# kalekundert/addapt

Measured on AMD Instinct MI355X. Metric: MC steps/sec (fold+score+accept), 100-nt sgRNA, 4096 walkers, 1/8 GPU, higher is better.
Workload: dtype i16x2; 1 GPU; BASELINE configs[1] (MFE-fold score only): default objective (apo: not active, holo: active; THEO aptamer 0.32 uM), 4 minimum-free-energy folds per scored step, synthetic 100-nt sgRNA template (SURVEY.md 8d), 4096 walkers per GPU, annealing 5 to 0 in 300 steps; fold=mfe, bppm=False, walkers_per_gpu=4096, global_walkers=4096, length=100, parallelism=walker-sharded x1 (no data-path collective)

## Files before the change

addapt_amd/csrc/mfe_pair.hip:

```cpp
#include <hip/hip_runtime.h>

#include <algorithm>
#include <cstdint>
#include <cstdio>
#include <cstdlib>
#include <utility>

#include "dev_types.hpp"
#include "fold_common.hpp"
#include "launch.hpp"
#include "mfe_common.hpp"

namespace adx {

#define PSTAMP(k) ADX_STAMP_AT(k)
#ifdef ADX_STAMP
#define PSTAMP_PARAMS , unsigned long long *st_acc, unsigned long long &st_last
#define PSTAMP_ARGS , st_acc, st_last
__device__ unsigned long long g_stamps_p[16][16];
__device__ unsigned long long g_stamps_pe[16][16];
#else
#define PSTAMP_PARAMS
#define PSTAMP_ARGS
#endif
// ... 145 lines not shown
        if (!ok[q]) continue;
        L.cc[off(d, N) + i - 1] = static_cast<uint8_t>(rtype(ty[q]) * 25 + (wjp[q] & 7) * 5 + (wim[q] & 7));
        u32 h = INF16;
        if (((wi1[q] >> 8) & 255) >= uint32_t(u)) {
            h = padd(hv[q], f1[q]);
            if (u == 3 || u == 4 || u == 6) {
                const int sh = special_hp(spk, hp_key(L.S, i, u + 2));
                if (sh >= 0) h = spv[sh];
            }
        }
        if (d == mL - 1 && mL > 0 && mt[q]) h = pmin(h, mextra);
        if (inb[q]) {
            L.qbm[off(d, N) + i - 1] = pr[q] ? h : MARK16;
            L.qm1[colb(j) + i - 1] = pr[q] ? f2[q] : INF16;
        }
    }
}

template <int NT, int NM>
__device__ __forceinline__ void pair_constants(const DevScaled *__restrict__ XS, const DevTables *__restrict__ TT,
                                               const CP &L) {
    static_assert(NT >= 288 && NT >= MFE_E4_SLOTS * 4, "one table element per thread");
    const int tid = threadIdx.x;
    const u32 *gct = reinterpret_cast<const u32 *>(XS->ctab);
    constexpr int NCT = (CT_SIZE + NT - 1) / NT;
    u32 v_ct[NCT];
#pragma unroll
    for (int t = 0; t < NCT; t++) v_ct[t] = gct[min(tid + t * NT, CT_SIZE - 1)];
    const DevTables &T0 = *TT;
    const u32 v_mh = __float_as_uint((&T0.mmH[0][0][0])[min(tid, 199)]);
    const u32 v_mi = __float_as_uint((&T0.mmI[0][0][0])[min(tid, 199)]);
    const u32 v_ms = __float_as_uint((&T0.mlstem[0][0][0])[min(tid, 199)]);
    const u32 v_ex = __float_as_uint((&T0.ext[0][0][0])[min(tid, 287)]);
    const u32 v_tau = __float_as_uint(T0.termAU[tid & 7]);
    const int ke = min(tid, MFE_E4_SLOTS * 4 - 1);
    const int e4a = MFE_E4_A[ke >> 2][ke & 3], e4u = MFE_E4_U[ke >> 2];
    const u32 v_e4 = XS->ku16[e4u][max(e4a, 0)];
#pragma unroll
    for (int t = 0; t < NCT; t++)
        if (tid + t * NT < CT_SIZE) L.ct[tid + t * NT] = v_ct[t];
    if (tid < 200) {
        L.dt[DT_MMH + tid] = v_mh;
        L.dt[DT_MMI + tid] = v_mi;
        L.dt[DT_MLS + tid] = v_ms;
    }
    if (tid < 288) L.dt[DT_EXT + tid] = v_ex;
    if (tid < 8) L.dt[DT_TAU + tid] = v_tau;
    if (tid < MFE_E4_SLOTS * 4) L.e4[tid] = e4a < 0 ? INF16 : v_e4;
    for (int k = tid; k < NM - 3; k += NT) {
        (L.qbm - (NM - 3))[k] = INF16;
        (L.cc - (NM - 3))[k] = 0;
    }
}

template <int NT, int NM>
__device__ __forceinline__ bool pair_setup(const KArgs &ka, const DevScaled *__restrict__ XS,
                                           const DevTables *__restrict__ TT, const int *vs, const uint8_t *raw,
                                           const CP &L, const IncM &inc, const int tid,
                                           unsigned long long *sst) {
    static_assert(NT == NWV * WAVE, "one wave per block slot");
    DevVariant V = ka.variants[vs[0]];
    V.ctx = uni(V.ctx), V.cons_off = uni(V.cons_off);
    const bool mh0 = uni(V.motif) != 0, mh1 = uni(ka.variants[vs[1]].motif) != 0;
    const int N = uni(V.N);
    const int lane = tid & (WAVE - 1);
    const int wid = uni(tid / WAVE);
    const int NP = L.np;
#ifdef ADX_STAMP
    const unsigned long long st_setup0 = __builtin_amdgcn_s_memtime();
#endif
    const Band bd = inc.band(N);
    const bool incr = bd.incr;
    const int m_lo = bd.m_lo;

    static_assert(NT >= MAX_SPECIAL_HP && NT >= MAX_MOTIF && NT >= NM + 2, "one setup element per thread");
    const u32 v_hp = __float_as_uint(XS->hp[min(tid, N)]);
    const int n_sp = uni(XS->n_special);
    const uint32_t v_spk = XS->sp_key[min(tid, MAX_SPECIAL_HP - 1)];
    const u32 v_spv = __float_as_uint(XS->sp_val[min(tid, MAX_SPECIAL_HP - 1)]);
    const uint8_t v_mc = XS->motif_code[min(tid, MAX_MOTIF - 1)];
    const int8_t v_mp = XS->motif_pt[min(tid, MAX_MOTIF - 1)];
    const uint8_t *cons = ka.cons + V.cons_off;
    const int np = N + 2;
    const int kp = min(tid, np - 1);
    uint8_t v_sw, v_up, v_dn, v_pt, v_en, v_fl;
    {
        const uint8_t *bef = nullptr, *aft = nullptr;
        int blen = 0;
        if (V.ctx >= 0) {
            bef = ka.ctx_seq + ka.ctx_off[4 * V.ctx + 0];
            blen = ka.ctx_off[4 * V.ctx + 1];
            aft = ka.ctx_seq + ka.ctx_off[4 * V.ctx + 2];
        }
        const int pp = (kp == 0 ? N : (kp == N + 1 ? 1 : kp)) - 1;
        const uint8_t *sp = pp < blen ? bef + pp : (pp < blen + ka.Nraw ? raw + (pp - blen) : aft + (pp - blen - ka.Nraw));
        v_sw = *sp;
        v_up = cons[kp];
        v_dn = cons[np + kp];
        v_pt = cons[2 * np + kp];
        v_en = cons[3 * np + kp];
        v_fl = cons[4 * np + kp];
    }
    if (tid < np) {
        L.S[tid] = v_sw;
        L.up[tid] = v_up;
        L.dn[tid] = v_dn;
        L.ptn[tid] = v_pt;
        L.enc[tid] = v_en;
        L.flg[tid] = v_fl;
        L.mat[tid] = 0;
        L.pos[tid] = u32(v_sw) | (u32(v_fl & 7) << 3) | (u32(v_up) << 8) | (u32(v_pt) << 16) | (u32(v_en) << 24);
    }
    const bool cst = tid >= 1 && tid <= N && (v_fl || v_pt);
    u32 *hpf = L.colmin;
    static_assert(4 * (NM + 2) >= NM + 1, "hairpin factors fit the U slots");
    if (tid <= N) hpf[tid] = v_hp;
    uint32_t *spk = reinterpret_cast<uint32_t *>(L.part);
    u32 *spv = spk + MAX_SPECIAL_HP;
    uint8_t *mcode = reinterpret_cast<uint8_t *>(spk + 2 * MAX_SPECIAL_HP);
    int8_t *mpt = reinterpret_cast<int8_t *>(mcode + MAX_MOTIF);
    static_assert(2 * MAX_SPECIAL_HP * 4 + 2 * MAX_MOTIF <= PLay<NM>::MLA - PLay<NM>::PART, "setup tables fit the partials");
    if (tid < MAX_SPECIAL_HP) {
        const bool on = tid < n_sp;
        spk[tid] = on ? v_spk : 0xFFFFFFFFu;
        spv[tid] = on ? v_spv : INF16;
    }
    if (tid < MAX_MOTIF) {
        mcode[tid] = v_mc;
        mpt[tid] = v_mp;
    }

    constexpr int CNM = ((NM - 4) * (NM - 3)) >> 1;
    constexpr int RS = (3 * (CNM >> 1) + NT - 1) / NT;
    const int Crs = ((N - 4) * (N - 3)) >> 1, half = Crs >> 1;
    uint2 rsv[RS];
    constexpr int RC = (((CNM + 15) >> 4) + NT - 1) / NT;
    const int C16 = (Crs + 15) >> 4;
    uint4 rcv[RC];
    u32 rod = 0, r5 = 0;
    if (incr) {
        const size_t Cs = size_t(ka.cells);
        const size_t gap = Cs - size_t(2 * half);
#pragma unroll
        for (int t = 0; t < RS; t++) {
            const int k = tid + t * NT;
            const int kk = k < 3 * half ? k : 0;
            const size_t o = size_t(2 * kk) + (kk >= half ? gap : 0) + (kk >= 2 * half ? gap : 0);
            rsv[t] = *reinterpret_cast<const uint2 *>(inc.src + o);
        }
#pragma unroll
        for (int t = 0; t < RC; t++) {
            const int k = tid + t * NT;
            rcv[t] = inc.cc_src[k < C16 ? k : 0];
        }
        rod = inc.src[min(tid, 2) * Cs + max(Crs - 1, 0)];
        r5 = inc.src[3 * Cs + min(tid, N)];
    } else {
        const int C = ((N - 4) * (N - 3)) >> 1;
        for (int k = tid; k < C; k += NT) L.qm[k] = INF16;
    }
#ifdef ADX_STAMP
    const unsigned long long st_s1 = __builtin_amdgcn_s_memtime();
#endif
    const bool constrained = block_or(L.flag, cst);
    const int mL = uni(XS->motif_len);
#ifdef ADX_STAMP
    const unsigned long long st_s2 = __builtin_amdgcn_s_memtime();
#endif
    if ((mh0 || mh1) && mL > 0) {
        for (int o0 = 1 + wid * WAVE; o0 + mL - 1 <= N; o0 += NT) {
            const int o = o0 + lane;
            const bool in = o + mL - 1 <= N;
            bool ok = in;
            for (int k0 = 0; k0 < mL; k0 += 8) {
                uint32_t sb[8], mb[8];
#pragma unroll
                for (int t = 0; t < 8; t++) {
                    sb[t] = L.S[min(o + k0 + t, N + 1)];
                    mb[t] = mcode[k0 + t];
                }
#pragma unroll
                for (int t = 0; t < 8; t++) ok = ok && (k0 + t >= mL || sb[t] == mb[t]);
                if (__ballot(ok) == 0) break;
            }
            if (in) L.mat[o] = ok ? 1 : 0;
        }
        __syncthreads();
        motif_constraints(L, mpt, mL, N, wid, lane);
    }
#ifdef ADX_STAMP
    const unsigned long long st_s25 = __builtin_amdgcn_s_memtime();
#endif
    if (incr) {
        static_assert(PLay<NM>::QM - PLay<NM>::QBM == PLay<NM>::QM1 - PLay<NM>::QM, "one stride between the tables");
        const int gapl = int((PLay<NM>::QM - PLay<NM>::QBM) / 4) - 2 * half;
#pragma unroll
        for (int t = 0; t < RS; t++) {
            const int k = tid + t * NT;
            if (k < 3 * half) {
                const int o = 2 * k + (k >= half ? gapl : 0) + (k >= 2 * half ? gapl : 0);
                *reinterpret_cast<uint2 *>(L.qbm + o) = rsv[t];
            }
        }
        if ((Crs & 1) && tid < 3) (tid == 0 ? L.qbm : tid == 1 ? L.qm : L.qm1)[Crs - 1] = rod;
#pragma unroll
        for (int t = 0; t < RC; t++) {
            const int k = tid + t * NT;
            if (k < C16) reinterpret_cast<uint4 *>(L.cc)[k] = rcv[t];
        }
        if (tid <= m_lo - 2 && tid <= N) L.q5[tid] = r5;
    }
    static_assert(NM - 4 <= 2 * WAVE, "the diagonals' quarter-set counts in two lane-sets");
    static_assert((NM - 4) + ((NM - 4) * (NM - 3) / 2 + 15) / 16 <= 6 * (NM + 2), "quarter-sets fit the split slots");
    u32 *qtab = L.mla;
    int tot = 0;
#pragma unroll
    for (int xs = 0; xs < 2; xs++) {
        const int d = 4 + xs * WAVE + lane;
        const int n = d <= N - 1 ? max(0, bd.chi(d) - bd.clo(d) + 1) : 0;
        const int q = (n + 15) >> 4;
        int v = q;
#pragma unroll
        for (int o = 1; o < WAVE; o <<= 1) {
            const int t = __shfl_up(v, o, WAVE);
            if (lane >= o) v += t;
        }
        if (wid == xs)
            for (int c = 0; c < q; c++) qtab[tot + v - q + c] = u32(d) | (u32(bd.clo(d) + 16 * c) << 8);
        tot += __shfl(v, WAVE - 1, WAVE);
    }
    tot = uni(tot);
    __syncthreads();
    const u32 mx = u32(uni(int(__float_as_uint(XS->motif_extra))));
    const u32 mextra = (mh0 ? (mx & 0xFFFFu) : 0x7FFFu) | (mh1 ? (mx & 0xFFFF0000u) : 0x7FFF0000u);
    if (tid == 0) q5_start(L, N);
#ifdef ADX_STAMP
    const unsigned long long st_s3 = __builtin_amdgcn_s_memtime();
#endif
    for (int I0 = wid * 4; 4 * I0 < tot; I0 += NWV * 4)
        cell_pass(L, bd, lane, I0, qtab, tot, hpf, spk, spv, mL, mextra);
#ifdef ADX_STAMP
    const unsigned long long st_s35 = __builtin_amdgcn_s_memtime();
#endif
    __syncthreads();
#ifdef ADX_STAMP
    const unsigned long long st_s4 = __builtin_amdgcn_s_memtime();
#endif
    for (int k = tid; k < 4 * 2 * NP; k += NT) L.part[k] = PINF;
    for (int k = tid; k < 6 * NP; k += NT) L.mla[k] = INF16;
    for (int k = tid; k < 4 * NP; k += NT) L.colmin[k] = INF16;
    __syncthreads();
#ifdef ADX_STAMP
    {
        const unsigned long long st_end = __builtin_amdgcn_s_memtime();
        sst[0] = st_end - st_setup0;
        sst[1] = st_s1 - st_setup0;
        sst[2] = st_s2 - st_s1;
        sst[3] = st_s25 - st_s2;
        sst[4] = st_s3 - st_s25;
        sst[5] = st_s4 - st_s3;
        sst[6] = st_s35 - st_s3;
    }
#endif
    return constrained;
}

__device__ __forceinline__ void build_list(const CP &L, const Band &bd, int lane, int db, int sl) {
    const int N = bd.N, NP2 = 2 * L.np;
    int base = 0, P0 = 0;
    for (int k = 0; k < 2; k++) {
        const int dn = db + k;
        if (k == 1) P0 = base;
        if (dn < 8 || dn > N - 1) continue;
        const int lo = bd.clo(dn), hi = bd.chi(dn);
        const int Ln = lanesets(hi - lo + 1);
        for (int ls = 0; ls < Ln; ls++) {
            const int i = lo + ls * WAVE + lane;
            const bool pr = i <= hi && L.qbm[off(dn, N) + i - 1] != MARK16;
            const uint64_t m = __ballot(pr);
            const int rk = base + __builtin_amdgcn_mbcnt_hi(uint32_t(m >> 32), __builtin_amdgcn_mbcnt_lo(uint32_t(m), 0u));
            if (pr) L.cl[sl * NP2 + rk] = uint8_t(i);
            if (pr && rk < WAVE) {
                const int j = i + dn;
                const int oc = brec_code(L, i, j);
                const u32 mmo = L.dt[DT_MMI + oc];
                u32 *rr = L.rec + sl * 2 * WAVE + rk;
                rr[0] = brec_word(i, oc, L.up[i + 1], L.dn[j - 1]);
                rr[WAVE] = (mmo & 0xFFFFu) | (padd(L.ct[CT_ONEN + oc], mmo) << 16);
            }
            base += __popcll(m);
        }
    }
    if (lane == 0) L.cnt[sl] = P0 | (base << 16);
}
__device__ __forceinline__ void load_list(const CP &L, int lane, int sl, int &PP, u32 &wd, u32 &mm) {
    PP = L.cnt[sl];
    const u32 *rr = L.rec + sl * 2 * WAVE + (lane & 15);
    wd = rr[0];
    mm = rr[WAVE];
}

struct FRun {
    int ab;
    int fd;
    int oE0, oE1, oS1, oS2, oS3;
    uint32_t mS, mM;
    uint32_t cW;
    int fI;
    uint32_t fSi, fSi1, fUi, fUi1;
    uint32_t fRq;
    uint32_t fJ4, fSj, fQ1;
};

template <int NM, int fls>
__device__ __forceinline__ void finalize(const CP &L, FRun &f, const BUni &U, int N, int d, int lane, int mloF,
                                         int mhiF, u32 mlclosing, u32 mlbase PSTAMP_PARAMS) {
    static_assert(NM - 4 <= 2 * WAVE - 1, "two overlapping lane-sets reach every row from row 1");
    static_assert(PLay<NM>::NP == NM + 2 && 4 * (NM + 2) * 4 < 65536, "slot strides as ds offsets");
    const uint32_t aqm = lds_addr(L.qm), aqm1 = lds_addr(L.qm1);
    const int e0 = d - 2, e1 = d - 1;
    const int R = N - e0;
    const int fr = max(1, mloF - 2 - e1);
    const int lr = min(R, mhiF + 3);
    if (e0 <= N - 1 && (f.ab == 0 || fr < f.ab)) {
        f.ab = max(1, lr - (lr - fr < 64 ? 63 : 126));
        f.fd = 0;
    }
    if (e0 <= N - 1 && (fls == 0 || lr - f.ab > 63)) {
        __builtin_amdgcn_s_setprio(PRIO_ROLE);
        constexpr uint32_t NP4 = uint32_t(NM + 2) * 4u;
        const uint32_t aq = U.aq, ac = U.ac, aS = lds_addr(L.S);
        if (fls == 1 || f.fd != d) {
            f.fI = f.ab + fls * 63 + lane;
            const int ic = min(f.fI, N);
            f.fSi = L.S[ic], f.fSi1 = L.S[ic + 1], f.fUi = L.up[ic], f.fUi1 = L.up[ic + 1];
            f.fRq = aqm + uint32_t(rowb(f.fI, N) - 4) * 4u;
            const int jA = f.fI + e0;
            f.fJ4 = uint32_t(jA) * 4u;
            f.fSj = aS + uint32_t(jA - 1);
            f.fQ1 = aqm1 + uint32_t(colb(jA - 1) + f.fI - 1) * 4u;
            f.oE0 = off(e0, N), f.oE1 = off(e1, N);
            f.oS1 = off(max(e0 - 1, 3), N), f.oS2 = off(max(e0 - 2, 3), N), f.oS3 = off(max(e0 - 3, 3), N);
            f.mS = uint32_t(e0 % 6) * NP4, f.mM = uint32_t((e0 + 4) % 6) * NP4;
            f.cW = uint32_t(e0 & 3) * NP4;
            f.fd = d;
        }
        const int i = f.fI;
        const uint32_t i4 = uint32_t(i) * 4u;
        const uint32_t q1P = f.fQ1, q1A = q1P + (f.fJ4 - 20u), q1B = q1A + (f.fJ4 - 16u);
        if (i >= fr && i <= lr) {
        const bool own = lane < 63 || fls == 1 || lr - f.ab <= 63;
        const bool rowB = i <= R - 1;
        const bool ghost = i == mhiF + 3;
        const uint32_t qA = (aq + uint32_t(f.oE0 - 1) * 4u) + i4, qB = (aq + uint32_t(f.oE1 - 1) * 4u) + i4;
        const uint32_t pA = (lds_addr(L.part) + 2u * f.cW) + i4;
        const uint32_t uW = (lds_addr(L.colmin) + f.cW) + f.fJ4;
        const uint32_t gq = f.fRq + uint32_t(e0) * 4u;
        u32 initA, cceA, stA, pqA, mlA, spA, upA, a0, a1, vS3, cS3, vS3b, cS3b, vS2, cS2, vS2b, cS2b, vS1, cS1;
        u32 initB, cceB, stB, mlB, spB, b0, b1, gqA, gqB;
        uint32_t sjm, sj, sjp, ujA, ujB, djm, dj;
        const uint32_t si = f.fSi, si1 = f.fSi1, ui = f.fUi, ui1 = f.fUi1;
        {
            const uint32_t mA = (lds_addr(L.mla) + f.mM + 4u) + i4;
            const uint32_t sA = (lds_addr(L.mla) + f.mS) + i4;
            const uint32_t uA = (lds_addr(L.colmin) + 3u * NP4 - f.cW) + f.fJ4;
            asm volatile(
                "ds_read_b32 %[initA], %[qA]\n"
                "ds_read_u8 %[cceA], %[kA]\n"
                "ds_read_b32 %[stA], %[q1A]\n"
                "ds_read_b32 %[pqA], %[q1P]\n"
                "ds_read_b32 %[mlA], %[mA]\n"
                "ds_read_b32 %[spA], %[sA]\n"
                "ds_read_b32 %[upA], %[uA]\n"
                "ds_read_b32 %[a0], %[pA]\n"
                "ds_read_b32 %[a1], %[pA] offset:%[pst]\n"
                "ds_read_b32 %[initB], %[qB]\n"
                "ds_read_u8 %[cceB], %[kB]\n"
                "ds_read_b32 %[stB], %[q1B]\n"
                "ds_read_b32 %[mlB], %[mA] offset:%[pst]\n"
                "ds_read_b32 %[spB], %[sA] offset:%[pst]\n"
                "ds_read_b32 %[b0], %[pA] offset:%[pst2]\n"
                "ds_read_b32 %[b1], %[pA] offset:%[pst3]\n"
                "ds_read_b32 %[vS3], %[q3]\n"
                "ds_read_b32 %[vS3b], %[q3] offset:4\n"
                "ds_read_b32 %[vS2], %[q2]\n"
                "ds_read_b32 %[vS2b], %[q2] offset:4\n"
                "ds_read_b32 %[vS1], %[q1]\n"
                "ds_read_u8 %[cS3], %[k3]\n"
                "ds_read_u8 %[cS3b], %[k3] offset:1\n"
                "ds_read_u8 %[cS2], %[k2]\n"
                "ds_read_u8 %[cS2b], %[k2] offset:1\n"
                "ds_read_u8 %[cS1], %[k1]\n"
                "ds_read_u8 %[sjm], %[aSj] offset:0\n"
                "ds_read_u8 %[sj], %[aSj] offset:1\n"
                "ds_read_u8 %[sjp], %[aSj] offset:2\n"
                "ds_read_u8 %[ujA], %[aSj] offset:%[ou0]\n"
                "ds_read_u8 %[ujB], %[aSj] offset:%[ou1]\n"
                "ds_read_u8 %[djm], %[aSj] offset:%[od0]\n"
                "ds_read_u8 %[dj], %[aSj] offset:%[od1]\n"
                "ds_read_b32 %[gqA], %[gq]\n"
                "ds_read_b32 %[gqB], %[gq] offset:4\n"
                "s_waitcnt lgkmcnt(0)"
                : [initA] "=&v"(initA), [cceA] "=&v"(cceA), [stA] "=&v"(stA), [pqA] "=&v"(pqA), [mlA] "=&v"(mlA),
                  [spA] "=&v"(spA), [upA] "=&v"(upA), [a0] "=&v"(a0), [a1] "=&v"(a1), [initB] "=&v"(initB),
                  [cceB] "=&v"(cceB), [stB] "=&v"(stB), [mlB] "=&v"(mlB), [spB] "=&v"(spB), [b0] "=&v"(b0),
                  [b1] "=&v"(b1), [vS3] "=&v"(vS3), [vS3b] "=&v"(vS3b), [vS2] "=&v"(vS2), [vS2b] "=&v"(vS2b),
                  [vS1] "=&v"(vS1), [cS3] "=&v"(cS3), [cS3b] "=&v"(cS3b), [cS2] "=&v"(cS2), [cS2b] "=&v"(cS2b),
                  [cS1] "=&v"(cS1), [sjm] "=&v"(sjm), [sj] "=&v"(sj), [sjp] "=&v"(sjp), [ujA] "=&v"(ujA),
                  [ujB] "=&v"(ujB), [djm] "=&v"(djm), [dj] "=&v"(dj), [gqA] "=&v"(gqA), [gqB] "=&v"(gqB)
                : [qA] "v"(qA), [kA] "v"((ac + uint32_t(f.oE0 - 1)) + uint32_t(i)), [q1A] "v"(q1A), [q1P] "v"(q1P),
                  [mA] "v"(mA), [sA] "v"(sA), [uA] "v"(uA), [pA] "v"(pA), [pst] "i"(NP4), [pst2] "i"(2 * NP4),
                  [pst3] "i"(3 * NP4), [qB] "v"(qB), [kB] "v"((ac + uint32_t(f.oE1 - 1)) + uint32_t(i)), [q1B] "v"(q1B),
                  [q3] "v"((aq + uint32_t(f.oS3) * 4u) + i4), [q2] "v"((aq + uint32_t(f.oS2) * 4u) + i4),
                  [q1] "v"((aq + uint32_t(f.oS1) * 4u) + i4), [k3] "v"((ac + uint32_t(f.oS3)) + uint32_t(i)),
                  [k2] "v"((ac + uint32_t(f.oS2)) + uint32_t(i)), [k1] "v"((ac + uint32_t(f.oS1)) + uint32_t(i)),
                  [aSj] "v"(f.fSj), [ou0] "i"(NM + 2 + 1), [ou1] "i"(NM + 2 + 2), [od0] "i"(2 * (NM + 2)),
                  [od1] "i"(2 * (NM + 2) + 1), [gq] "v"(gq)
                : "memory");
        }
#ifdef ADX_STAMP_F
        PSTAMP(11);
#endif
        static_assert(NM + 2 == PLay<NM>::NP, "partial halves are NP words apart");
        const int tyA = ptype(si, sj), tyB = ptype(si, sjp);
        const int t8A = tyA * 8, t8B = tyB * 8;
        auto stk = [&](u32 v, u32 c, int t8) {
            return padd(v, padd(L.ct[CT_INVMM + c], L.ct[CT_STK + t8 + ((int(c) * 41) >> 10)]));
        };
        u32 iA = INF16, iB = INF16;
        if (e0 >= 6) iA = stk(vS2, cS2, t8A);
        if (e0 >= 7) {
            iA = pmin(iA, djm >= 1 ? padd(stk(vS3, cS3, t8A), U.fs1) : INF16);
            iA = pmin(iA, ui1 >= 1 ? padd(stk(vS3b, cS3b, t8A), U.fs1) : INF16);
        }
        if (e1 >= 6) iB = stk(vS1, cS1, t8B);
        if (e1 >= 7) {
            iB = pmin(iB, dj >= 1 ? padd(stk(vS2, cS2, t8B), U.fs1) : INF16);
            iB = pmin(iB, ui1 >= 1 ? padd(stk(vS2b, cS2b, t8B), U.fs1) : INF16);
        }
        const u32 mlclA = padd(mlclosing, L.dt[DT_MLS + rtype(tyA) * 25 + sjm * 5 + si1]);
        const u32 mlclB = padd(mlclosing, L.dt[DT_MLS + rtype(tyB) * 25 + sj * 5 + si1]);
        const u32 mmiA = L.dt[DT_MMI + cceA], mmiB = L.dt[DT_MMI + cceB];
        const bool inA = i >= mloF - 1 - e0 && i <= mhiF + 1;
        const bool inB = rowB && e1 <= N - 1 && i >= mloF - 1 - e1 && i <= mhiF + 1;
        auto st32 = [](uint32_t a, u32 v) { *lds_at<u32>(a) = v; };
        u32 m1A = stA;
        if (inA) {
            const u32 prev = (e0 >= 5 && ujA >= 1) ? padd(pqA, mlbase) : INF16;
            u32 f1 = prev;
            if (initA != MARK16) {
                u32 c = pmin(initA, pack2(int(a0), int(a1)));
                c = pmin(c, iA);
                c = pfin(pmin(c, padd(mlA, mlclA)));
                if (own) st32(qA, pfin(padd(c, mmiA)));
                f1 = pmin(padd(c, stA), prev);
            }
            m1A = pfin(f1);
            if (own) st32(q1A, m1A);
        }
        const u32 UA = ghost ? gqA : (ui >= 1 ? pmin(m1A, padd(upA, mlbase)) : m1A);
        u32 m1B = stB;
        if (inB) {
            const u32 prev = (e1 >= 5 && ujB >= 1) ? padd(m1A, mlbase) : INF16;
            u32 f1 = prev;
            if (initB != MARK16) {
                u32 c = pmin(initB, pack2(int(b0), int(b1)));
                c = pmin(c, iB);
                c = pfin(pmin(c, padd(mlB, mlclB)));
                if (own) st32(qB, pfin(padd(c, mmiB)));
                f1 = pmin(padd(c, stB), prev);
            }
            m1B = pfin(f1);
            if (own) st32(q1B, m1B);
        }
#ifdef ADX_STAMP_F
        PSTAMP(12);
#endif
        const u32 UA1 = u32(__builtin_amdgcn_ds_bpermute((lane + 1) * 4, int(UA)));
        const u32 UB = ghost ? gqB : (ui >= 1 ? pmin(m1B, padd(UA1, mlbase)) : m1B);
        if (own) {
            st32(uW, UA);
            st32(pA, u32(PINF));
            st32(pA + NP4, u32(PINF));
            if (e0 <= N - 3 && i >= mloF - 2 - e0 && i <= min(R, mhiF + 2))
                st32(gq, pfin(pmin(e0 >= 9 ? spA : INF16, UA)));
        }
        if (own && rowB && e1 <= N - 1) {
            st32(uW + NP4 + 4u, UB);
            st32(pA + 2u * NP4, u32(PINF));
            st32(pA + 3u * NP4, u32(PINF));
            if (e1 <= N - 3 && i >= mloF - 2 - e1 && i <= min(R - 1, mhiF + 2))
                st32(gq + 4u, pfin(pmin(e1 >= 9 ? spB : INF16, UB)));
        }
#ifdef ADX_STAMP_F
        PSTAMP(13);
#endif
        }
#ifdef ADX_STAMP_F
        {
            const uint64_t on = __ballot(i >= fr && i <= lr);
            if (on != 0) {
                const int src = __ffsll((long long)on) - 1;
                auto from = [&](unsigned long long v) {
                    const uint32_t lo = __builtin_amdgcn_readlane(uint32_t(v), src);
                    const uint32_t hi = __builtin_amdgcn_readlane(uint32_t(v >> 32), src);
                    return (unsigned long long)lo | ((unsigned long long)hi << 32);
                };
                st_acc[11] = from(st_acc[11]), st_acc[12] = from(st_acc[12]), st_acc[13] = from(st_acc[13]);
                st_last = from(st_last);
            }
        }
#endif
        if constexpr (fls == 0) {
        f.fQ1 = q1B;
        f.fJ4 += 8u, f.fSj += 2u;
        f.oS3 = f.oS1, f.oS2 = f.oE0, f.oS1 = f.oE1;
        f.oE0 = f.oE1 + (N - e1), f.oE1 = f.oE0 + (N - e1 - 1);
        f.mM = f.mS, f.mS = f.mS == 4u * NP4 ? 0u : f.mS + 2u * NP4;
        f.cW ^= 2u * NP4;
        f.fd = d + 2;
        }
        __builtin_amdgcn_s_setprio(0);
    }
}

__device__ __forceinline__ int slices(int P) { return P <= 16 ? 2 : (P <= 32 ? 1 : 0); }
__device__ __forceinline__ u32 lo2(u32 x) { return __builtin_amdgcn_perm(x, x, 0x05040504u); }
__device__ __forceinline__ u32 hi2(u32 x) { return __builtin_amdgcn_perm(x, x, 0x07060706u); }

template <int blk>
__device__ __forceinline__ void block_partials(const CP &L, const DevTables &T, BUni &U, int d, int lane, int sl, int cPP,
                                               u32 cwd, u32 cmm, bool constrained, u32 tauE, u32 fsm5 PSTAMP_PARAMS) {
    const int N = U.N, NP = L.np, NP2 = 2 * NP;
    const uint32_t ae4 = lds_addr(L.e4);
    if (d + 1 >= 8 && d <= N - 1) {
        const int P0 = uni(cPP & 0xFFFF), P = uni(cPP >> 16);
        const int sh = slices(P);
        const int cwl = 6 - sh;
        const int Lb = (P + (1 << cwl) - 1) >> cwl;
        const int r = lane >> cwl;
        U.d = d;
        U.umax = d - 5 < 30 ? d - 5 : 30;
        for (int ls = 0; ls < Lb && blk < MFE_NBLK; ls++) {
            const int idx = (ls << cwl) + (lane & ((1 << cwl) - 1));
            if (idx < P) {
                const int hb = idx >= P0 ? 1 : 0;
                const int dd = d + hb;
                BRec c;
                if (ls == 0 && sh == 2) {
                    c = brec_unpack(cwd, lo2(cmm), hi2(cmm));
                } else if (idx < WAVE) {
                    const u32 *rr = L.rec + sl * 2 * WAVE + idx;
                    c = brec_unpack(rr[0], lo2(rr[WAVE]), hi2(rr[WAVE]));
                } else {
                    const int i = L.cl[sl * NP2 + idx];
                    c = brec_of(L, i, i + dd);
                }
                const int i = c.i, oc = c.oc, type = (oc * 41) >> 10;
                const int uml = dd - 6 < 30 ? dd - 6 : 30;
                BCell C;
                C.i = i + hb * (N - d + 2);
                C.hb = hb;
                C.ty8 = type * 8;
                bcell_slice(C, r, sh, ae4);
                C.A = c.A;
                C.B = c.B;
                const u32 tau = type > 2 ? tauE : 0u;
                auto has = [&](unsigned bits) { return ((bits >> (sh * 8 + blk)) & 1u) != 0; };
                C.m23f = has(size_bits(5)) ? padd(L.ct[CT_M23O + oc], fsm5) : INF16;
                C.t11 = C.t12 = C.t21 = C.t22 = INF16;
                bcell_tables(C, L, T, N, dd, i, oc, uml, has(size_bits(2)), has(size_bits(3)), has(size_bits(4)));
                Acc a{INF16, INF16, INF16, INF16, INF16, INF16};
                const bool mk = constrained && __ballot(C.A < uml || C.B < uml) != 0;
                U.mk = mk;
                PSTAMP(9);
                if (sh == 2) mfe_block_s4(blk, U, C, a);
                else if (sh == 1) mfe_block_s2(blk, U, C, a);
                else mfe_block(blk, U, C, a);
                PSTAMP(10);
                const u32 acc = acc_fold(a, C, sh, c.mmo, c.mo, tau);
                if (r == 0) {
                    int *pp = L.part + (dd & 3) * 2 * NP + i;
                    atomicMin(pp, sext_lo(acc));
                    atomicMin(pp + NP, sext_hi(acc));
                }
            }
        }
    }
}

template <int NR>
__device__ __forceinline__ void split_chunk(const CP &L, int N, int i, int j, int Tt, int t0, u32 &sp0, u32 &sp1) {
    const uint32_t aqm = lds_addr(L.qm), aqm1 = lds_addr(L.qm1);
    u32 av[NR], rv[NR];
    const uint32_t pa = aqm1 + uint32_t(colb(j) + i - 1 + t0) * 4u;
    const uint32_t pr = aqm + uint32_t(rowb(i, N) - 5 + t0) * 4u;
    if constexpr (NR == 16) {
        asm volatile(
                "ds_read_b32 %0, %32 offset:0\n"
                "ds_read_b32 %1, %32 offset:4\n"
                "ds_read_b32 %2, %32 offset:8\n"
                "ds_read_b32 %3, %32 offset:12\n"
                "ds_read_b32 %4, %32 offset:16\n"
                "ds_read_b32 %5, %32 offset:20\n"
                "ds_read_b32 %6, %32 offset:24\n"
                "ds_read_b32 %7, %32 offset:28\n"
                "ds_read_b32 %8, %32 offset:32\n"
                "ds_read_b32 %9, %32 offset:36\n"
                "ds_read_b32 %10, %32 offset:40\n"
                "ds_read_b32 %11, %32 offset:44\n"
                "ds_read_b32 %12, %32 offset:48\n"
                "ds_read_b32 %13, %32 offset:52\n"
                "ds_read_b32 %14, %32 offset:56\n"
                "ds_read_b32 %15, %32 offset:60\n"
                "ds_read_b32 %16, %33 offset:0\n"
                "ds_read_b32 %17, %33 offset:4\n"
                "ds_read_b32 %18, %33 offset:8\n"
                "ds_read_b32 %19, %33 offset:12\n"
                "ds_read_b32 %20, %33 offset:16\n"
                "ds_read_b32 %21, %33 offset:20\n"
                "ds_read_b32 %22, %33 offset:24\n"
                "ds_read_b32 %23, %33 offset:28\n"
                "ds_read_b32 %24, %33 offset:32\n"
                "ds_read_b32 %25, %33 offset:36\n"
                "ds_read_b32 %26, %33 offset:40\n"
                "ds_read_b32 %27, %33 offset:44\n"
                "ds_read_b32 %28, %33 offset:48\n"
                "ds_read_b32 %29, %33 offset:52\n"
                "ds_read_b32 %30, %33 offset:56\n"
                "ds_read_b32 %31, %33 offset:60\n"
            "s_waitcnt lgkmcnt(0)"
            : "=&v"(av[0]), "=&v"(av[1]), "=&v"(av[2]), "=&v"(av[3]), "=&v"(av[4]), "=&v"(av[5]), "=&v"(av[6]), "=&v"(av[7]), "=&v"(av[8]), "=&v"(av[9]), "=&v"(av[10]), "=&v"(av[11]), "=&v"(av[12]), "=&v"(av[13]), "=&v"(av[14]), "=&v"(av[15]), "=&v"(rv[0]), "=&v"(rv[1]), "=&v"(rv[2]), "=&v"(rv[3]), "=&v"(rv[4]), "=&v"(rv[5]), "=&v"(rv[6]), "=&v"(rv[7]), "=&v"(rv[8]), "=&v"(rv[9]), "=&v"(rv[10]), "=&v"(rv[11]), "=&v"(rv[12]), "=&v"(rv[13]), "=&v"(rv[14]), "=&v"(rv[15])
            : "v"(pa), "v"(pr)
            : "memory");
    } else if constexpr (NR == 4) {
        asm volatile(
                "ds_read_b32 %0, %8 offset:0\n"
                "ds_read_b32 %1, %8 offset:4\n"
                "ds_read_b32 %2, %8 offset:8\n"
                "ds_read_b32 %3, %8 offset:12\n"
                "ds_read_b32 %4, %9 offset:0\n"
                "ds_read_b32 %5, %9 offset:4\n"
                "ds_read_b32 %6, %9 offset:8\n"
                "ds_read_b32 %7, %9 offset:12\n"
            "s_waitcnt lgkmcnt(0)"
            : "=&v"(av[0]), "=&v"(av[1]), "=&v"(av[2]), "=&v"(av[3]), "=&v"(rv[0]), "=&v"(rv[1]), "=&v"(rv[2]), "=&v"(rv[3])
            : "v"(pa), "v"(pr)
            : "memory");
    } else {
        asm volatile(
                "ds_read_b32 %0, %16 offset:0\n"
                "ds_read_b32 %1, %16 offset:4\n"
                "ds_read_b32 %2, %16 offset:8\n"
                "ds_read_b32 %3, %16 offset:12\n"
                "ds_read_b32 %4, %16 offset:16\n"
                "ds_read_b32 %5, %16 offset:20\n"
                "ds_read_b32 %6, %16 offset:24\n"
                "ds_read_b32 %7, %16 offset:28\n"
                "ds_read_b32 %8, %17 offset:0\n"
                "ds_read_b32 %9, %17 offset:4\n"
                "ds_read_b32 %10, %17 offset:8\n"
                "ds_read_b32 %11, %17 offset:12\n"
                "ds_read_b32 %12, %17 offset:16\n"
                "ds_read_b32 %13, %17 offset:20\n"
                "ds_read_b32 %14, %17 offset:24\n"
                "ds_read_b32 %15, %17 offset:28\n"
            "s_waitcnt lgkmcnt(0)"
            : "=&v"(av[0]), "=&v"(av[1]), "=&v"(av[2]), "=&v"(av[3]), "=&v"(av[4]), "=&v"(av[5]), "=&v"(av[6]), "=&v"(av[7]), "=&v"(rv[0]), "=&v"(rv[1]), "=&v"(rv[2]), "=&v"(rv[3]), "=&v"(rv[4]), "=&v"(rv[5]), "=&v"(rv[6]), "=&v"(rv[7])
            : "v"(pa), "v"(pr)
            : "memory");
    }
    const int lim = Tt - t0;
    if (__ballot(lim < NR - 1) == 0) {
#pragma unroll
        for (int k = 0; k < NR; k += 2) {
            sp0 = pmin(sp0, padd(rv[k], av[k]));
            sp1 = pmin(sp1, padd(rv[k + 1], av[k + 1]));
        }
    } else {
#pragma unroll
        for (int k = 0; k < NR; k += 2) {
            sp0 = pmin(sp0, padd(rv[k], k <= lim ? av[k] : INF16));
            sp1 = pmin(sp1, padd(rv[k + 1], k + 1 <= lim ? av[k + 1] : INF16));
        }
    }
}

__device__ __forceinline__ void split_rows(const CP &L, const Band &bd, int s, int lane) {
    const int N = bd.N, NP = L.np;
    if (s < 9 || s > N - 3) return;
    __builtin_amdgcn_s_setprio(PRIO_ROLE);
    const int lo = bd.qlo(s), hi = bd.qhi(s);
    const int Lm = lanesets(hi - lo + 1);
    const int Tt = s - 4;
    u32 *slot = L.mla + (s % 6) * NP;
    for (int ls = 0; ls < Lm; ls++) {
        const int nc = min(WAVE, hi - lo + 1 - ls * WAVE);
        const int lc = nc <= 1 ? 0 : 32 - __clz(nc - 1);
        const int cst = 1 << lc, lsl = 6 - lc;
        const int c = lane & (cst - 1), rr = lane >> lc;
        int i = lo + ls * WAVE + c;
        const bool valid = c < nc;
        if (!valid) i = hi;
        const int j = i + s;
        const int nb = Tt - 4;
        const int bs = nb > 0 ? (nb + (1 << lsl) - 1) >> lsl : 0;
        u32 sp0 = INF16, sp1 = INF16;
        int t0 = 5 + rr * bs;
        for (int ch = 0; ch < (bs >> 4); ch++, t0 += 16) split_chunk<16>(L, N, i, j, Tt, t0, sp0, sp1);
        const int rem = bs & 15;
        if (rem > 8) split_chunk<16>(L, N, i, j, Tt, t0, sp0, sp1);
        else if (rem > 4) split_chunk<8>(L, N, i, j, Tt, t0, sp0, sp1);
        else if (rem > 0) split_chunk<4>(L, N, i, j, Tt, t0, sp0, sp1);
        u32 split = pmin(sp0, sp1);
        for (int k = cst; k < WAVE; k <<= 1) split = pmin(split, u32(__shfl_xor(int(split), k, WAVE)));
        if (valid && rr == 0) slot[i] = pfin(split);
    }
    __builtin_amdgcn_s_setprio(0);
}

__device__ __forceinline__ void q5_columns(const CP &L, const Band &bd, int d, int lane) {
    const int N = bd.N, m_lo = bd.m_lo;
    const bool incr = bd.incr;
    const int j0 = d - 3, j1 = d - 2;
    const bool w0 = j0 >= 5 && j0 <= N && (!incr || j0 >= m_lo - 1);
    const bool w1 = j1 >= 5 && j1 <= N && (!incr || j1 >= m_lo - 1);
    if (w0 || w1) {
        __builtin_amdgcn_s_setprio(PRIO_ROLE);
        const int j1r = j1 <= N ? j1 : N;
        const int s0 = L.S[j0], s1 = L.S[j1r];
        const int sp0 = (j0 < N) ? L.S[j0 + 1] : 5, sp1 = (j1r < N) ? L.S[j1r + 1] : 5;
        u32 acc0 = INF16, acc1 = INF16;
        for (int k0 = 1; k0 <= j1r - 4; k0 += WAVE) {
            const int kk = k0 + lane;
            const bool ok1 = kk <= j1r - 4, ok0 = kk <= j0 - 4;
            const int k = ok1 ? kk : 1;
            const int sk = L.S[k], skm = (k > 1) ? L.S[k - 1] : 5;
            const u32 q5k = L.q5[k - 1];
            const int ix1 = off(j1r - k, N) + k - 1;
            const int ix0 = off(max(j0 - k, 4), N) + k - 1;
            const u32 ex1 = L.dt[DT_EXT + ptype(sk, s1) * 36 + skm * 6 + sp1];
            const u32 ex0 = L.dt[DT_EXT + ptype(sk, s0) * 36 + skm * 6 + sp0];
            const u32 t1 = padd(padd(q5k, L.qbm[ix1]), padd(L.ct[CT_INVMM + L.cc[ix1]], ex1));
            const u32 t0 = padd(padd(q5k, L.qbm[ix0]), padd(L.ct[CT_INVMM + L.cc[ix0]], ex0));
            acc1 = pmin(acc1, ok1 ? t1 : INF16);
            acc0 = pmin(acc0, ok0 ? t0 : INF16);
        }
        const u32 red0 = wave_min(acc0), red1 = wave_min(acc1);
        if (lane == 0) {
            u32 q0 = L.q5[j0];
            if (w0) {
                q0 = pfin(pmin((L.up[j0] >= 1) ? L.q5[j0 - 1] : INF16, red0));
                L.q5[j0] = q0;
            }
            if (w1) L.q5[j1] = pfin(pmin((L.up[j1] >= 1) ? q0 : INF16, red1));
        }
        __builtin_amdgcn_s_setprio(0);
    }
}

template <int NT, int NM, int WID>
__device__ __forceinline__ void mfe_pair_fold(const KArgs &ka, const DevScaled *__restrict__ XS,
                                              const DevTables *__restrict__ TT, const int *vs, const CP &L,
                                              const IncM &inc, const bool constrained, const int lane,
                                              const unsigned long long *sst) {
    const DevVariant V = ka.variants[vs[0]];
    const int N = uni(V.N);
    constexpr int wid = WID;
    constexpr int fls = FW[0] == wid ? 0 : (FW[1] == wid ? 1 : -1);
    const u32 *gct = reinterpret_cast<const u32 *>(XS->ctab);
    const Band bd = inc.band(N);
    const u32 mlclosing = u32(uni(int(__float_as_uint(XS->mlclosing))));
    const u32 mlbase = u32(uni(int(__float_as_uint(XS->mlbase_sig))));
    const u32 tauE = u32(uni(int(gct[CT_FSM + 6])));
    const u32 fsm5 = u32(uni(int(gct[CT_FSM + 5])));
    BUni U = buni(L, XS, N);
    U.fs1 = u32(uni(int(U.fs1)));
    if (wid == L_WAVE) {
        if (lane == 0) L.cnt[0] = 0;
        build_list(L, bd, lane, 8, 1);
    }
    __syncthreads();
    int cPP = 0;
    u32 cwd = 0, cmm = 0;

#ifdef ADX_STAMP
    unsigned long long st_acc[16] = {0, 0, 0, 0, 0, 0, 0, 0, 0, 0, 0, 0, 0, 0, 0, 0};
    const unsigned long long st_sw0 = __builtin_amdgcn_s_memtime();
    unsigned long long st_last = st_sw0;
#ifndef ADX_STAMP_F
    st_acc[11] = sst[1];
    st_acc[12] = sst[2];
    st_acc[13] = sst[3];
#endif
    st_acc[7] = sst[4];
    st_acc[14] = sst[5];
    st_acc[15] = sst[6];
    st_acc[8] = sst[0] + (st_last - st_sw0);
#endif
// ... 188 lines not shown
```

Before: 2.462 million MC steps/s.

## Pack two diagonals into one wave when finalize span fits 32 lanes

When the active row range of the MFE finalize step spans at most 32 rows, the wave is split into two half-waves. Each half handles one of the two diagonals (e0 and e1) at the same time, instead of one wave-wide pass that computes both diagonals serially per lane. Cross-half dependencies are resolved with permlane32_swap and ds_bpermute. This is meant to shorten the latency-bound serial per-lane path on narrow windows. The cost is extra lane-exchange instructions and an added branch, plus re-anchoring logic whenever the packing mode changes.

Measured after the change: 2.488 million MC steps/s, median of 6. +1.1%, better.

```diff
diff --git a/addapt_amd/csrc/mfe_pair.hip b/addapt_amd/csrc/mfe_pair.hip
--- a/addapt_amd/csrc/mfe_pair.hip
+++ b/addapt_amd/csrc/mfe_pair.hip
@@ -471,6 +471,7 @@
 
 struct FRun {
     int ab;
+    int pk;
     int fd;
     int oE0, oE1, oS1, oS2, oS3;
     uint32_t mS, mM;
@@ -479,7 +480,114 @@
     uint32_t fSi, fSi1, fUi, fUi1;
     uint32_t fRq;
     uint32_t fJ4, fSj, fQ1;
+    uint32_t fH;
 };
+
+template <int NM>
+__device__ __forceinline__ void finalize_packed(const CP &L, const FRun &f, const BUni &U, int N, int e0, int lane,
+                                                int mloF, int mhiF, u32 mlclosing, u32 mlbase, uint32_t q1P,
+                                                uint32_t q1 PSTAMP_PARAMS) {
+    constexpr uint32_t NP4 = uint32_t(NM + 2) * 4u;
+    const uint32_t aq = U.aq, ac = U.ac;
+    const bool hB = lane >= 32;
+    const int i = f.fI;
+    const uint32_t i4 = uint32_t(i) * 4u, iH = i4 + f.fH;
+    const int e = e0 + (hB ? 1 : 0);
+    const int j = int(f.fJ4 >> 2);
+    const int oE = hB ? f.oE1 : f.oE0;
+    const int o2 = hB ? f.oS1 : f.oS2, o3 = hB ? f.oS2 : f.oS3;
+    const bool cell = j <= N;
+    const bool ghost = i == mhiF + 3;
+    const uint32_t qX = (aq - 4u) + uint32_t(oE) * 4u + i4;
+    const uint32_t pA = (lds_addr(L.part) + 2u * f.cW) + iH + f.fH;
+    const uint32_t uW = (lds_addr(L.colmin) + f.cW) + f.fH + f.fJ4;
+    const uint32_t gq = f.fRq + (f.fJ4 - i4);
+    u32 init, cce, st, pq, ml, sp, up, p0, p1, v2, c2, v3, c3, v3b, c3b, gv;
+    uint32_t sjm, sj, uj, djm;
+    const uint32_t si = f.fSi, si1 = f.fSi1, ui = f.fUi, ui1 = f.fUi1;
+    {
+        const uint32_t mA = (lds_addr(L.mla) + f.mM + 4u) + iH;
+        const uint32_t sA = (lds_addr(L.mla) + f.mS) + iH;
+        const uint32_t uA = (lds_addr(L.colmin) + 3u * NP4 - f.cW) + f.fJ4;
+        asm volatile(
+            "ds_read_b32 %[init], %[qX]\n"
+            "ds_read_u8 %[cce], %[kX]\n"
+            "ds_read_b32 %[st], %[q1]\n"
+            "ds_read_b32 %[pq], %[q1P]\n"
+            "ds_read_b32 %[ml], %[mA]\n"
+            "ds_read_b32 %[sp], %[sA]\n"
+            "ds_read_b32 %[up], %[uA]\n"
+            "ds_read_b32 %[p0], %[pA]\n"
+            "ds_read_b32 %[p1], %[pA] offset:%[pst]\n"
+            "ds_read_b32 %[v2], %[q2]\n"
+            "ds_read_b32 %[v3], %[q3]\n"
+            "ds_read_b32 %[v3b], %[q3] offset:4\n"
+            "ds_read_u8 %[c2], %[k2]\n"
+            "ds_read_u8 %[c3], %[k3]\n"
+            "ds_read_u8 %[c3b], %[k3] offset:1\n"
+            "ds_read_u8 %[sjm], %[aSj] offset:0\n"
+            "ds_read_u8 %[sj], %[aSj] offset:1\n"
+            "ds_read_u8 %[uj], %[aSj] offset:%[ou]\n"
+            "ds_read_u8 %[djm], %[aSj] offset:%[od]\n"
+            "ds_read_b32 %[gv], %[gq]\n"
+            "s_waitcnt lgkmcnt(0)"
+            : [init] "=&v"(init), [cce] "=&v"(cce), [st] "=&v"(st), [pq] "=&v"(pq), [ml] "=&v"(ml), [sp] "=&v"(sp),
+              [up] "=&v"(up), [p0] "=&v"(p0), [p1] "=&v"(p1), [v2] "=&v"(v2), [v3] "=&v"(v3), [v3b] "=&v"(v3b),
+              [c2] "=&v"(c2), [c3] "=&v"(c3), [c3b] "=&v"(c3b), [sjm] "=&v"(sjm), [sj] "=&v"(sj), [uj] "=&v"(uj),
+              [djm] "=&v"(djm), [gv] "=&v"(gv)
+            : [qX] "v"(qX), [kX] "v"((ac - 1u) + uint32_t(oE) + uint32_t(i)), [q1] "v"(q1), [q1P] "v"(q1P), [mA] "v"(mA),
+              [sA] "v"(sA), [uA] "v"(uA), [pA] "v"(pA), [pst] "i"(NP4), [q2] "v"(aq + uint32_t(o2) * 4u + i4),
+              [q3] "v"(aq + uint32_t(o3) * 4u + i4), [k2] "v"(ac + uint32_t(o2) + uint32_t(i)),
+              [k3] "v"(ac + uint32_t(o3) + uint32_t(i)), [aSj] "v"(f.fSj), [ou] "i"(NM + 2 + 1),
+              [od] "i"(2 * (NM + 2)), [gq] "v"(gq)
+            : "memory");
+    }
+#ifdef ADX_STAMP_F
+    PSTAMP(11);
+#endif
+    const int ty = ptype(si, sj), t8 = ty * 8;
+    auto stk = [&](u32 v, u32 c) {
+        return padd(v, padd(L.ct[CT_INVMM + c], L.ct[CT_STK + t8 + ((int(c) * 41) >> 10)]));
+    };
+    u32 iX = e >= 6 ? stk(v2, c2) : INF16;
+    if (e0 >= 6) {
+        const bool b7 = e >= 7;
+        iX = pmin(iX, b7 && djm >= 1 ? padd(stk(v3, c3), U.fs1) : INF16);
+        iX = pmin(iX, b7 && ui1 >= 1 ? padd(stk(v3b, c3b), U.fs1) : INF16);
+    }
+    const u32 mlcl = padd(mlclosing, L.dt[DT_MLS + rtype(ty) * 25 + sjm * 5 + si1]);
+    const u32 mmi = L.dt[DT_MMI + cce];
+    const bool in = cell && j >= mloF - 1 && i <= mhiF + 1;
+    auto st32 = [](uint32_t a, u32 v) { *lds_at<u32>(a) = v; };
+    const bool pairable = init != MARK16;
+    u32 c = pmin(init, pack2(int(p0), int(p1)));
+    c = pmin(c, iX);
+    c = pfin(pmin(c, padd(ml, mlcl)));
+    if (in && pairable) st32(qX, pfin(padd(c, mmi)));
+    const u32 cs = pairable ? padd(c, st) : INF16;
+    const bool pv = e >= 5 && uj >= 1;
+    auto m1of = [&](u32 p) { return in ? pfin(pmin(cs, pv ? padd(p, mlbase) : INF16)) : st; };
+    u32 m1 = m1of(pq);
+    const auto sw = __builtin_amdgcn_permlane32_swap(pq, m1, false, false);
+    m1 = m1of(u32(sw[0]));
+    if (in) st32(q1, m1);
+#ifdef ADX_STAMP_F
+    PSTAMP(12);
+#endif
+    auto uof = [&](u32 below) { return ghost ? gv : (ui >= 1 ? pmin(m1, padd(below, mlbase)) : m1); };
+    const u32 UA1 = u32(__builtin_amdgcn_ds_bpermute(((lane & 31) + 1) * 4, int(uof(up))));
+    const u32 Uf = uof(hB ? UA1 : up);
+    if (cell) {
+        st32(uW, Uf);
+        st32(pA, u32(PINF));
+        st32(pA + NP4, u32(PINF));
+        if (e <= N - 3 && j >= mloF - 2 && i <= mhiF + 2)
+            st32(gq, pfin(pmin(e >= 9 ? sp : INF16, Uf)));
+    }
+#ifdef ADX_STAMP_F
+    PSTAMP(13);
+#endif
+}
 
 template <int NM, int fls>
 __device__ __forceinline__ void finalize(const CP &L, FRun &f, const BUni &U, int N, int d, int lane, int mloF,
@@ -491,8 +599,10 @@
     const int R = N - e0;
     const int fr = max(1, mloF - 2 - e1);
     const int lr = min(R, mhiF + 3);
-    if (e0 <= N - 1 && (f.ab == 0 || fr < f.ab)) {
-        f.ab = max(1, lr - (lr - fr < 64 ? 63 : 126));
+    const int fit = lr - fr <= 31 ? 1 : 0;
+    if (e0 <= N - 1 && (f.ab == 0 || fr < f.ab || fit != f.pk)) {
+        f.pk = fit;
+        f.ab = max(1, lr - (fit ? 31 : (lr - fr < 64 ? 63 : 126)));
         f.fd = 0;
     }
     if (e0 <= N - 1 && (fls == 0 || lr - f.ab > 63)) {
@@ -500,11 +610,14 @@
         constexpr uint32_t NP4 = uint32_t(NM + 2) * 4u;
         const uint32_t aq = U.aq, ac = U.ac, aS = lds_addr(L.S);
         if (fls == 1 || f.fd != d) {
-            f.fI = f.ab + fls * 63 + lane;
+            const bool pk = fls == 0 && f.pk != 0;
+            const int hB = pk && lane >= 32 ? 1 : 0;
+            f.fI = f.ab + (pk ? (lane & 31) : fls * 63 + lane);
+            f.fH = hB ? NP4 : 0u;
             const int ic = min(f.fI, N);
             f.fSi = L.S[ic], f.fSi1 = L.S[ic + 1], f.fUi = L.up[ic], f.fUi1 = L.up[ic + 1];
             f.fRq = aqm + uint32_t(rowb(f.fI, N) - 4) * 4u;
-            const int jA = f.fI + e0;
+            const int jA = f.fI + e0 + hB;
             f.fJ4 = uint32_t(jA) * 4u;
             f.fSj = aS + uint32_t(jA - 1);
             f.fQ1 = aqm1 + uint32_t(colb(jA - 1) + f.fI - 1) * 4u;
@@ -518,6 +631,11 @@
         const uint32_t i4 = uint32_t(i) * 4u;
         const uint32_t q1P = f.fQ1, q1A = q1P + (f.fJ4 - 20u), q1B = q1A + (f.fJ4 - 16u);
         if (i >= fr && i <= lr) {
+        bool pk = false;
+        if constexpr (fls == 0) pk = f.pk != 0;
+        if (pk) {
+            finalize_packed<NM>(L, f, U, N, e0, lane, mloF, mhiF, mlclosing, mlbase, q1P, q1A PSTAMP_ARGS);
+        } else {
         const bool own = lane < 63 || fls == 1 || lr - f.ab <= 63;
         const bool rowB = i <= R - 1;
         const bool ghost = i == mhiF + 3;
@@ -664,6 +782,7 @@
 #ifdef ADX_STAMP_F
         PSTAMP(13);
 #endif
+        }
         }
 #ifdef ADX_STAMP_F
         {
```
